# pasqal-io/pulser-diff

Measured on AMD Instinct MI355X. Metric: time-steps/sec (fwd+grad), higher is better.
Workload: dtype c128; 1 GPU; c3: 20-qubit register, 1000 time steps, fwd+grad wrt 8 pulse params per parameter set, KRYLOV_SE map, 1 parameter set(s) in the job; n_qubits=20, trajectories_total=1, trajectories_this_rank=1, ranks=1, gathered_parameter_sets=1, parallelism=trajectory-sharded x1 (one replica per rank), kernel_family=chained-tiles, tape=full

## Files before the change

pulser-diff_amd/csrc/pair_kernels.hpp:

```cpp
#pragma once

struct Chain2Args {
    const double2* v;
    const double2* w;
    const double2* t;
    double2* vmid_out;
    double2* y_out;
    double2* w_out;
    double2* t_out;
    const double* utt;
    const double* vr;
    const double* coef_fin;
    const double* coef_sta;
    long coef_bstride;
    double a_r, a_i, b_r, b_i, k_r, k_i;
    double g1_r, g1_i, b1_r, b1_i;
    int lo, hs, hb;
    uint32_t dim;
    int has_p, has_q;
    int gd;
    uint32_t fin_mask;
    uint32_t dmask[kMaxGroups];
    int dcnt[kMaxGroups];
    int b_first, b_count;
    const double* obs;
    double* expect_slot;
    int n_obs;
    long exp_ostride;
};

template <int LT, int LGT>
__global__ __launch_bounds__(1 << LGT) void k_chain2(Chain2Args a) {
    constexpr int NT = 1 << LGT, R = 1 << (LT - LGT);
    extern __shared__ __attribute__((aligned(16))) double2 tiles[];
    double* red = reinterpret_cast<double*>(tiles + 2 * (size_t(1) << LT));
    const unsigned tid = threadIdx.x;
    const unsigned t = blockIdx.x;
    const unsigned bl = blockIdx.y;
    if (bl >= unsigned(a.b_count)) return;
    const unsigned bt = unsigned(a.b_first) + bl;
    const size_t boff = size_t(bt) * a.dim;
    const unsigned lomask = (1u << a.lo) - 1u;
    const int midlow = a.hs - a.lo;
    const unsigned xbase = ((t & ((1u << midlow) - 1u)) << a.lo) | ((t >> midlow) << (a.hs + a.hb));
    double2 uu[R], ww[R], tt[R];
    unsigned xg[R];
#pragma unroll
    for (int r = 0; r < R; ++r) {
        const unsigned i = unsigned(r) * NT + tid;
        xg[r] = xbase | (i & lomask) | ((i >> a.lo) << a.hs);
        uu[r] = stream_load(a.v + boff + xg[r]);
    }
#pragma unroll
    for (int r = 0; r < R; ++r) ww[r] = stream_load(a.w + boff + xg[r]);
#pragma unroll
    for (int r = 0; r < R; ++r) tt[r] = stream_load(a.t + boff + xg[r]);
    double du[R];
    {
        const double* __restrict__ vrow = a.vr + size_t(t) * 16;
        double vloc[LT];
#pragma unroll
        for (int b2 = 0; b2 < LT; ++b2) vloc[b2] = vrow[b2];
        double dlane = vrow[LT];
#pragma unroll
        for (int b2 = 0; b2 < LGT; ++b2)
            if (!(tid >> b2 & 1u)) dlane += vloc[b2];
#pragma unroll
        for (int r = 0; r < R; ++r) {
            double d = a.utt[unsigned(r) * NT + tid] + dlane;
#pragma unroll
            for (int b2 = LGT; b2 < LT; ++b2)
                if (!(r >> (b2 - LGT) & 1)) d += vloc[b2];
            du[r] = d;
        }
    }
    auto diag = [&](const double* cf, int r) -> double {
        double d = du[r];
        for (int g = 0; g < a.gd; ++g) d += cf[2 + g] * double(a.dcnt[g] - popc_i(xg[r] & a.dmask[g]));
        return d;
    };
    int buf = 0;
    auto put = [&](const double2 (&val)[R]) -> const double2* {
        double2* tile = tiles + (size_t(buf) << LT);
#pragma unroll
        for (int r = 0; r < R; ++r) tile[unsigned(r) * NT + tid] = val[r];
        __syncthreads();
        buf ^= 1;
        return tile;
    };
    auto cmul = [](double xr, double xi, const double2& z) { return make_double2(xr * z.x - xi * z.y, xr * z.y + xi * z.x); };

    double2 y[R];
    if (a.has_p) {
        const double* __restrict__ cf = a.coef_fin + bt * a.coef_bstride;
        const double c = cf[0];
        double2 s[R], h1[R], ds[R];
        partner_sums<LT, LGT, false>(put(uu), uu, a.fin_mask, tid, s, ds);
        double d[R];
#pragma unroll
        for (int r = 0; r < R; ++r) {
            d[r] = diag(cf, r);
            h1[r].x = d[r] * uu[r].x + c * (ww[r].x + s[r].x);
            h1[r].y = d[r] * uu[r].y + c * (ww[r].y + s[r].y);
            const double2 p = cmul(a.a_r, a.a_i, uu[r]), q = cmul(a.b_r, a.b_i, h1[r]);
            y[r] = make_double2(p.x + q.x, p.y + q.y);
        }
        if (a.vmid_out) {
#pragma unroll
            for (int r = 0; r < R; ++r) {
                const double2 p = cmul(a.g1_r, a.g1_i, uu[r]), q = cmul(a.b1_r, a.b1_i, h1[r]);
                stream_store(a.vmid_out + boff + xg[r], make_double2(p.x + q.x, p.y + q.y));
            }
        }
        if (a.k_r != 0.0 || a.k_i != 0.0) {
            double2 e[R], pe[R];
#pragma unroll
            for (int r = 0; r < R; ++r) e[r] = make_double2(h1[r].x + c * ww[r].x, h1[r].y + c * ww[r].y);
            partner_sums<LT, LGT, false>(put(e), e, a.fin_mask, tid, pe, ds);
#pragma unroll
            for (int r = 0; r < R; ++r) {
                const double2 z = make_double2(d[r] * h1[r].x + c * (tt[r].x + pe[r].x), d[r] * h1[r].y + c * (tt[r].y + pe[r].y));
                const double2 k = cmul(a.k_r, a.k_i, z);
                y[r].x += k.x;
                y[r].y += k.y;
            }
        }
#pragma unroll
        for (int r = 0; r < R; ++r) stream_store(a.y_out + boff + xg[r], y[r]);
        if (a.obs) {
            for (int o = 0; o < a.n_obs; ++o) {
                double ex = 0.0;
#pragma unroll
                for (int r = 0; r < R; ++r) ex += a.obs[size_t(o) * a.dim + xg[r]] * (y[r].x * y[r].x + y[r].y * y[r].y);
                wg_atomic_add<NT>(ex, a.expect_slot + o * a.exp_ostride + bt, red);
            }
        }
    } else {
#pragma unroll
        for (int r = 0; r < R; ++r) y[r] = uu[r];
    }
    if (!a.has_q) return;

    const double* __restrict__ cf = a.coef_sta + bt * a.coef_bstride;
    const double c = cf[0];
    double2 w2[R], ds[R];
    partner_sums<LT, LGT, false, true>(put(y), y, ~0u, tid, w2, ds);
#pragma unroll
    for (int r = 0; r < R; ++r) stream_store(a.w_out + boff + xg[r], w2[r]);
    double2 z[R];
#pragma unroll
    for (int r = 0; r < R; ++r) {
        const double d = diag(cf, r);
        z[r] = make_double2(d * y[r].x + c * w2[r].x, d * y[r].y + c * w2[r].y);
    }
    double2 t2[R];
    partner_sums<LT, LGT, false, true>(put(z), z, ~0u, tid, t2, ds);
#pragma unroll
    for (int r = 0; r < R; ++r) stream_store(a.t_out + boff + xg[r], t2[r]);
}

struct Chain2BwdArgs {
    const double2* mu;
    const double2* w;
    const double2* t;
    const double2* xa;
    const double2* xb;
    double2* mu_out;
    double2* w_out;
    double2* t_out;
    const double* utt;
    const double* vr;
    const double* coef_fin;
    const double* coef_sta;
    long coef_bstride;
    double gb_r, gb_i, bb_r, bb_i;
    double k_r, k_i;
    double ga_r, ga_i, ba_r, ba_i;
    double cba_r, cba_i, cbb_r, cbb_i;
    int lo, hs, hb;
    uint32_t dim;
    int has_p, has_q;
    int gd;
    uint32_t fin_mask;
    uint32_t dmask;
    int dcnt;
    int b_first, b_count;
    double* ge_fin;
    long ge_bstride, ge_rstride;
    int det_slot;
    double* wtot;
    const double2* inj_gstate;
    const double* inj_gexp;
    const double* inj_obs;
    int inj_n_obs;
    long inj_ostride;
};

template <int LT, int LGT>
__global__ __launch_bounds__(1 << LGT) void k_chain2_bwd(Chain2BwdArgs a) {
    constexpr int NT = 1 << LGT, R = 1 << (LT - LGT), NW = NT / 64;
    extern __shared__ __attribute__((aligned(16))) double2 tiles[];
    double* red = reinterpret_cast<double*>(tiles + 2 * (size_t(1) << LT));
    const unsigned tid = threadIdx.x;
    const unsigned t = blockIdx.x;
    const unsigned bl = blockIdx.y;
    if (bl >= unsigned(a.b_count)) return;
    const unsigned bt = unsigned(a.b_first) + bl;
    const size_t boff = size_t(bt) * a.dim;
    const unsigned lomask = (1u << a.lo) - 1u;
    const int midlow = a.hs - a.lo;
    const unsigned xbase = ((t & ((1u << midlow) - 1u)) << a.lo) | ((t >> midlow) << (a.hs + a.hb));
    if (tid < 2 * NW) red[tid] = 0.0;
    double2 uu[R], ww[R], xa[R], xb[R], tp[R];
    unsigned xg[R];
    auto reindex = [&]() {
        unsigned tid_o = tid;
        asm volatile("" : "+v"(tid_o));
#pragma unroll
        for (int r = 0; r < R; ++r) {
            const unsigned i = unsigned(r) * NT + tid_o;
            xg[r] = xbase | (i & lomask) | ((i >> a.lo) << a.hs);
        }
    };
#pragma unroll
    for (int r = 0; r < R; ++r) {
        const unsigned i = unsigned(r) * NT + tid;
        xg[r] = xbase | (i & lomask) | ((i >> a.lo) << a.hs);
        uu[r] = stream_load(a.mu + boff + xg[r]);
    }
#pragma unroll
    for (int r = 0; r < R; ++r) ww[r] = stream_load(a.w + boff + xg[r]);
#pragma unroll
    for (int r = 0; r < R; ++r) xa[r] = stream_load(a.xa + boff + xg[r]);
    auto interaction_diagonal = [&](double (&du)[R]) {
        unsigned tid_o = tid;
        asm volatile("" : "+v"(tid_o));
        const double* __restrict__ vrow = a.vr + size_t(t) * 16;
        double vloc[LT];
#pragma unroll
        for (int b2 = 0; b2 < LT; ++b2) vloc[b2] = vrow[b2];
        double dlane = vrow[LT];
#pragma unroll
        for (int b2 = 0; b2 < LGT; ++b2)
            if (!(tid >> b2 & 1u)) dlane += vloc[b2];
#pragma unroll
        for (int r = 0; r < R; ++r) {
            double d = a.utt[unsigned(r) * NT + tid_o] + dlane;
#pragma unroll
            for (int b2 = LGT; b2 < LT; ++b2)
                if (!(r >> (b2 - LGT) & 1)) d += vloc[b2];
            du[r] = d;
        }
    };
    double du[R];
    interaction_diagonal(du);
    auto cnt = [&](int r) -> double { return a.gd ? double(a.dcnt - popc_i(xg[r] & a.dmask)) : 0.0; };
    int buf = 0;
    auto put = [&](const double2 (&val)[R]) -> const double2* {
        double2* tile = tiles + (size_t(buf) << LT);
#pragma unroll
        for (int r = 0; r < R; ++r) tile[unsigned(r) * NT + tid] = val[r];
        __syncthreads();
        buf ^= 1;
        return tile;
    };
    auto cmul = [](double xr, double xi, const double2& z) { return make_double2(xr * z.x - xi * z.y, xr * z.y + xi * z.x); };
    auto cdot = [](const double2& p, const double2& x) { return make_double2(p.x * x.x + p.y * x.y, p.x * x.y - p.y * x.x); };

    double2 y[R];
    if (a.has_p) {
        const double* __restrict__ cf = a.coef_fin + bt * a.coef_bstride;
        const double c = cf[0], cdet = a.gd ? cf[2] : 0.0;
        double2 pm[R], mid[R];
        double wx[R];
        double zc = 0.0;
        const bool two = a.k_r != 0.0 || a.k_i != 0.0;
        {
            double2* etile = tiles + (size_t(buf ^ 1) << LT);
#pragma unroll
            for (int r = 0; r < R; ++r) etile[unsigned(r) * NT + tid] = xa[r];
            double2 s[R], ds[R];
            partner_sums<LT, LGT, false>(put(uu), uu, a.fin_mask, tid, s, ds);
#pragma unroll
            for (int r = 0; r < R; ++r) {
                const double2 xav = etile[unsigned(r) * NT + tid];
                const double d = du[r] + cdet * cnt(r);
                pm[r] = make_double2(ww[r].x + s[r].x, ww[r].y + s[r].y);
                const double2 h1 = make_double2(d * uu[r].x + c * pm[r].x, d * uu[r].y + c * pm[r].y);
                if (two) etile[unsigned(r) * NT + tid] = make_double2(h1.x + c * ww[r].x, h1.y + c * ww[r].y);
                const double2 q1 = cdot(pm[r], xav);
                zc += a.cba_r * q1.x - a.cba_i * q1.y;
                const double2 wa = cdot(uu[r], xav);
                wx[r] = a.cba_r * wa.x - a.cba_i * wa.y;
                const double2 mm = cmul(a.ga_r, a.ga_i, uu[r]), mh = cmul(a.ba_r, a.ba_i, h1);
                mid[r] = make_double2(mm.x + mh.x, mm.y + mh.y);
            }
        }
        park1<NW>(zc, red, 0);
        zc = 0.0;
#pragma unroll
        for (int r = 0; r < R; ++r) xb[r] = stream_load(a.xb + boff + xg[r]);
#pragma unroll
        for (int r = 0; r < R; ++r) tp[r] = stream_load(a.t + boff + xg[r]);
        reindex();
        double sgd = 0.0;
#pragma unroll
        for (int r = 0; r < R; ++r) {
            const double2 wb = cdot(mid[r], xb[r]);
            const double wr = wx[r] + (a.cbb_r * wb.x - a.cbb_i * wb.y);
            if (a.wtot) unsafeAtomicAdd(a.wtot + xg[r], wr);
            sgd += wr * cnt(r);
            const double2 gpm = cmul(a.ga_r, a.ga_i, pm[r]);
            const double2 q = cdot(gpm, xb[r]);
            zc += a.cbb_r * q.x - a.cbb_i * q.y;
            const double d = du[r] + cdet * cnt(r);
            const double2 y1 = cmul(a.gb_r + a.bb_r * d, a.gb_i + a.bb_i * d, mid[r]), y2 = cmul(a.bb_r * c, a.bb_i * c, gpm);
            y[r] = make_double2(y1.x + y2.x, y1.y + y2.y);
        }
        __builtin_amdgcn_sched_barrier(0);
        if (two) {
            __syncthreads();
            buf ^= 1;
        }
        if (two) {
            const double2* tile = tiles + (size_t(buf ^ 1) << LT);
#pragma unroll
            for (int b = 0; b < LT; ++b) {
                if (a.fin_mask >> b & 1u) {
#pragma unroll
                    for (int r = 0; r < R; ++r) {
                        const double2 q = tile[(unsigned(r) * NT + tid) ^ (1u << b)];
                        tp[r].x += q.x;
                        tp[r].y += q.y;
                    }
                }
            }
        }
        const double kc_r = a.k_r * c, kc_i = a.k_i * c;
#pragma unroll
        for (int r = 0; r < R; ++r) {
            const double2 kt = cmul(kc_r, kc_i, tp[r]);
            y[r].x += kt.x;
            y[r].y += kt.y;
            const double2 q = cdot(cmul(a.ba_r, a.ba_i, tp[r]), xb[r]);
            zc += a.cbb_r * q.x - a.cbb_i * q.y;
        }
        park2<NW>(zc, sgd, red, 0, 1);
        reindex();
        if (a.inj_gexp || a.inj_gstate) {
            if (a.inj_gexp) {
                bool any = false;
                for (int o = 0; o < a.inj_n_obs; ++o) any |= a.inj_gexp[o * a.inj_ostride + bt] != 0.0;
                if (any) {
#pragma unroll
                    for (int r = 0; r < R; ++r) {
                        double wsum = 0.0;
                        for (int o = 0; o < a.inj_n_obs; ++o) wsum += a.inj_gexp[o * a.inj_ostride + bt] * a.inj_obs[size_t(o) * a.dim + xg[r]];
                        y[r].x += 2.0 * wsum * xb[r].x;
                        y[r].y += 2.0 * wsum * xb[r].y;
                    }
                }
            }
            if (a.inj_gstate) {
#pragma unroll
                for (int r = 0; r < R; ++r) {
                    const double2 gs = stream_load(a.inj_gstate + boff + xg[r]);
                    y[r].x += gs.x;
                    y[r].y += gs.y;
                }
            }
        }
#pragma unroll
        for (int r = 0; r < R; ++r) stream_store(a.mu_out + boff + xg[r], y[r]);
    } else {
#pragma unroll
        for (int r = 0; r < R; ++r) y[r] = uu[r];
    }
    auto flush = [&]() {
        if (a.has_p && tid < 2) {
            double sum = 0.0;
#pragma unroll
            for (int w = 0; w < NW; ++w) sum += red[tid * NW + w];
            double* ge = a.ge_fin + bt * a.ge_bstride + (blockIdx.x % kGradReplicas) * a.ge_rstride;
            if (sum != 0.0) unsafeAtomicAdd(ge + (tid ? a.det_slot : 0), sum);
        }
    };
    if (!a.has_q) {
        __syncthreads();
        flush();
        return;
    }

    const double* __restrict__ cf = a.coef_sta + bt * a.coef_bstride;
    const double c = cf[0], cdet = a.gd ? cf[2] : 0.0;
    reindex();
    interaction_diagonal(du);
    double2 w2[R], ds[R];
    partner_sums<LT, LGT, false, true>(put(y), y, ~0u, tid, w2, ds);
#pragma unroll
    for (int r = 0; r < R; ++r) stream_store(a.w_out + boff + xg[r], w2[r]);
    double2 z[R];
#pragma unroll
    for (int r = 0; r < R; ++r) {
        const double d = du[r] + cdet * cnt(r);
        z[r] = make_double2(d * y[r].x + c * w2[r].x, d * y[r].y + c * w2[r].y);
    }
    double2 t2[R];
    partner_sums<LT, LGT, false, true>(put(z), z, ~0u, tid, t2, ds);
#pragma unroll
    for (int r = 0; r < R; ++r) stream_store(a.t_out + boff + xg[r], t2[r]);
    flush();
}
```

pulser-diff_amd/csrc/pair_launch.hpp:

```cpp
#pragma once

namespace {

bool pair_legal(const Runtime& rt) {
    const Plan& pl = rt.pl;
    const uint32_t all = uint32_t(pl.dim) - 1u;
    const ChainGeom g = chain_geom(rt);
    return rt.pair_mode >= 0 && rt.variant == 0 && !rt.force_three && !rt.force_xcd && chain_enabled(rt) && !pl.shard_bits &&
           pl.N > kTileBits && pl.N <= 20 && g.lt == kTileBits && g.layouts == 2 && pl.ga.n == 1 && pl.gd.n <= 1 && !pl.ga.flagged &&
           (pl.ga.amp_index_mask[0] & all) == all && !(rt.flags & 1) && pl.off_pp2 && pl.off_pp3;
}

bool pair_enabled(const Runtime& rt) {
    if (!pair_legal(rt)) return false;
    return rt.pair_mode == 1 || (rt.pl.N == 20 && rt.pl.B == 1);
}

template <class Args>
void fill_chain2(Args& ca, const Runtime& rt, char* ws, const std::vector<ChainItem>& items, const std::vector<std::pair<int, int>>& blk,
                 int j, const double2* cur, const BatchSlice& bs) {
    const Plan& pl = rt.pl;
    double2* wt[2][2] = {{reinterpret_cast<double2*>(ws + pl.off_pp0), reinterpret_cast<double2*>(ws + pl.off_pp1)},
                         {reinterpret_cast<double2*>(ws + pl.off_pp2), reinterpret_cast<double2*>(ws + pl.off_pp3)}};
    const ChainGeom geom{kTileBits, 2};
    const int nb = int(blk.size()), L = j & 1;
    const LayoutDesc Y = chain_layout(pl.NL, L, geom), X = chain_layout(pl.NL, L ^ 1, geom);
    ca.w = j ? wt[(j - 1) & 1][0] : cur;
    ca.t = j ? wt[(j - 1) & 1][1] : cur;
    ca.utt = split_tables(pl, ws, kTileBits) + size_t(L) * rt.per_layout(kTileBits);
    ca.vr = ca.utt + (size_t(1) << kTileBits);
    ca.coef_bstride = rt.coef_bstride();
    ca.coef_fin = rt.coef(ws, j ? items[blk[j - 1].first].stage : 0);
    ca.coef_sta = rt.coef(ws, j < nb ? items[blk[j].first].stage : 0);
    ca.lo = Y.lo;
    ca.hs = Y.hs;
    ca.hb = Y.hb;
    ca.dim = uint32_t(pl.dim);
    ca.has_p = j > 0;
    ca.has_q = j < nb;
    ca.gd = pl.gd.n;
    ca.b_first = bs.first;
    ca.b_count = bs.count;
    if (ca.has_p) ca.fin_mask = to_tile_mask(Y, kTileBits, uint32_t(pl.dim - 1) & ~X.bits);
    if (ca.has_q) {
        ca.w_out = wt[j & 1][0];
        ca.t_out = wt[j & 1][1];
    }
}

template <int LGT>
int launch_chain2_t(const Chain2Args& ca, unsigned tiles, hipStream_t stream) {
    constexpr int LT = kTileBits;
    const size_t lds = 2 * (size_t(1) << LT) * sizeof(double2) + 256;
    if (int rc = set_max_dynamic_lds_once<&k_chain2<LT, LGT>>(lds)) return rc;
    hipLaunchKernelGGL((k_chain2<LT, LGT>), dim3(tiles, unsigned(ca.b_count)), dim3(1 << LGT), lds, stream, ca);
    LAUNCH_CHECK();
    return RYDIFF_OK;
}

template <class DstFn, class DoneFn, class ExpFn>
int run_chain2(const Runtime& rt, char* ws, const std::vector<ChainItem>& items, const double2* start, DstFn dst, bool keep_mid,
               DoneFn on_done, ExpFn exp_slot, const BatchSlice& bs, hipStream_t stream) {
    const Plan& pl = rt.pl;
    const int F = int(items.size());
    if (F <= 0) return RYDIFF_OK;
    std::vector<std::pair<int, int>> blk;
    for (int i = 0; i < F;) {
        if (i + 1 < F && items[i + 1].stage == items[i].stage) {
            blk.push_back({i, i + 1});
            i += 2;
        } else {
            blk.push_back({i, -1});
            ++i;
        }
    }
    const unsigned tiles = unsigned(pl.dim >> kTileBits);
    const int nb = int(blk.size());
    const double2* cur = start;
    for (int j = 0; j <= nb; ++j) {
        Chain2Args ca{};
        fill_chain2(ca, rt, ws, items, blk, j, cur, bs);
        ca.v = cur;
        fill_detuning(ca.dmask, ca.dcnt, pl);
        int f0 = -1, last = -1;
        if (ca.has_p) {
            f0 = blk[j - 1].first;
            const int f1 = blk[j - 1].second;
            last = f1 >= 0 ? f1 : f0;
            const FactorScalars& s1 = items[f0].s;
            const FactorScalars s2 = f1 >= 0 ? items[f1].s : FactorScalars{1.0, 0.0, 0.0, 0.0};
            const std::complex<double> g1(s1.gr, s1.gi), b1(s1.br, s1.bi), g2(s2.gr, s2.gi), b2(s2.br, s2.bi);
            const std::complex<double> qa = g1 * g2, qb = g1 * b2 + b1 * g2, qk = b1 * b2;
            ca.a_r = qa.real();
            ca.a_i = qa.imag();
            ca.b_r = qb.real();
            ca.b_i = qb.imag();
            ca.k_r = qk.real();
            ca.k_i = qk.imag();
            ca.g1_r = s1.gr;
            ca.g1_i = s1.gi;
            ca.b1_r = s1.br;
            ca.b1_i = s1.bi;
            ca.vmid_out = (f1 >= 0 && keep_mid) ? dst(f0) : nullptr;
            ca.y_out = dst(last);
            if (!ca.y_out) return fail(RYDIFF_EINVAL, "internal: chain destination missing");
            ChainStep cs{};
            exp_slot(last, cs);
            ca.obs = cs.obs;
            ca.expect_slot = cs.expect_slot;
            ca.n_obs = cs.n_obs;
            ca.exp_ostride = cs.exp_ostride;
        }
        int rc = launch_chain2_t<10>(ca, tiles, stream);
        if (rc) return rc;
        if (ca.has_p) {
            if (ca.vmid_out) {
                rc = on_done(f0, ca.vmid_out);
                if (rc) return rc;
            }
            rc = on_done(last, ca.y_out);
            if (rc) return rc;
            cur = ca.y_out;
        }
    }
    return RYDIFF_OK;
}

bool pair_bwd_enabled(const Runtime& rt) {
    const ChainGeom g = chain_geom(rt);
    return !rt.pair_bwd_off && rt.real_amp_grad && pair_enabled(rt) && g.lt == kTileBits && g.layouts == 2;
}

template <int LGT>
int launch_chain2_bwd_t(const Chain2BwdArgs& ca, unsigned tiles, hipStream_t stream) {
    constexpr int LT = kTileBits;
    const size_t lds = 2 * (size_t(1) << LT) * sizeof(double2) + 2 * ((size_t(1) << LGT) / 64) * sizeof(double);
    if (int rc = set_max_dynamic_lds_once<&k_chain2_bwd<LT, LGT>>(lds)) return rc;
    hipLaunchKernelGGL((k_chain2_bwd<LT, LGT>), dim3(tiles, unsigned(ca.b_count)), dim3(1 << LGT), lds, stream, ca);
    LAUNCH_CHECK();
    return RYDIFF_OK;
}

template <class StageEndFn>
int run_chain2_bwd(const Runtime& rt, char* ws, const std::vector<ChainItem>& items, const std::vector<const double2*>& xs,
                   const std::vector<int>& save_k, const double2* lam_in, double2* lam_bufs[2], int& cl, double* wtot,
                   StageEndFn on_stage_end, const BatchSlice& bs, const InjectSource& inj, hipStream_t stream) {
    const Plan& pl = rt.pl;
    const int M = int(items.size());
    if (M <= 0) return RYDIFF_OK;
    std::vector<std::pair<int, int>> blk;
    for (int f = M - 1; f >= 0;) {
        if (f >= 1 && items[f - 1].stage == items[f].stage) {
            blk.push_back({f - 1, f});
            f -= 2;
        } else {
            blk.push_back({f, -1});
            --f;
        }
    }
    const unsigned tiles = unsigned(pl.dim >> kTileBits);
    const int nb = int(blk.size());
    const double2* cur = lam_in;
    int rc = on_stage_end(items[M - 1].stage, cur, xs[M]);
    if (rc) return rc;
    for (int j = 0; j <= nb; ++j) {
        Chain2BwdArgs ca{};
        fill_chain2(ca, rt, ws, items, blk, j, cur, bs);
        ca.mu = cur;
        ca.xa = ca.xb = cur;
        if (pl.gd.n) {
            ca.dmask = pl.gd.amp_index_mask[0];
            ca.dcnt = pl.gd.count[0];
        }
        ca.ge_fin = rt.ge(ws, 0);
        ca.ge_bstride = rt.ge_bstride();
        ca.ge_rstride = pl.NC + 1;
        ca.det_slot = 2 * pl.ga.n;
        ca.wtot = wtot;
        int fb = -1;
        if (ca.has_p) {
            fb = blk[j - 1].first;
            const int fa = blk[j - 1].second;
            const FactorScalars& sb = items[fb].s;
            const FactorScalars sa = fa >= 0 ? items[fa].s : FactorScalars{1.0, 0.0, 0.0, 0.0};
            const std::complex<double> gb(sb.gr, -sb.gi), bb(sb.br, -sb.bi), ga(sa.gr, -sa.gi), ba(sa.br, -sa.bi);
            const std::complex<double> qk = ba * bb;
            ca.gb_r = gb.real();
            ca.gb_i = gb.imag();
            ca.bb_r = bb.real();
            ca.bb_i = bb.imag();
            ca.k_r = qk.real();
            ca.k_i = qk.imag();
            ca.ga_r = ga.real();
            ca.ga_i = ga.imag();
            ca.ba_r = ba.real();
            ca.ba_i = ba.imag();
            ca.cba_r = sa.br;
            ca.cba_i = sa.bi;
            ca.cbb_r = sb.br;
            ca.cbb_i = sb.bi;
            ca.xb = xs[fb];
            ca.xa = fa >= 0 ? xs[fa] : xs[fb];
            ca.ge_fin = rt.ge(ws, items[fb].stage);
            cl ^= 1;
            ca.mu_out = lam_bufs[cl];
            if (ca.mu_out == cur) return fail(RYDIFF_EINVAL, "internal: cotangent ping-pong clash");
            fill_inject(ca, inj, save_k[fb], pl);
        }
        rc = launch_chain2_bwd_t<10>(ca, tiles, stream);
        if (rc) return rc;
        if (ca.has_p) {
            cur = ca.mu_out;
            if (fb >= 1 && items[fb].stage != items[fb - 1].stage) {
                rc = on_stage_end(items[fb - 1].stage, cur, xs[fb]);
                if (rc) return rc;
            }
        }
    }
    return RYDIFF_OK;
}

}
```

pulser-diff_amd/csrc/rydiff.hip:

```cpp
#include <hip/hip_runtime.h>

#include <algorithm>
#include <atomic>
#include <complex>
#include <cstdio>
#include <cstdlib>
#include <cstring>
#include <functional>
#include <mutex>
#include <type_traits>
#include <string>
#include <vector>

#include "../../include/rydiff.h"
#include "plan.hpp"
#include "poly.hpp"

using namespace rydiff;

#include "common.hpp"
#include "direct_kernels.hpp"
#include "chain_kernels.hpp"
#include "pair_kernels.hpp"
#include "persist_kernels.hpp"
#include "lane_kernels.hpp"
#include "pauli_kernels.hpp"
static_assert(sizeof(PersistFactor) == 48, "plan.hpp sizes the factor table with 48 bytes per entry");

#include "runtime.hpp"
#include "pauli_launch.hpp"
#include "direct_launch.hpp"
#include "chain_launch.hpp"
#include "pair_launch.hpp"
#include "persist_launch.hpp"

namespace {

void describe_kernels(const Runtime& rt, const RydProblem* p, bool backward, RydPlanInfo* info) {
    const Plan& pl = rt.pl;
    auto b = [](bool v) { return v ? "true" : "false"; };
    info->kernel_fwd[0] = info->kernel_bwd[0] = 0;
    if (info->kernel_family == 3) {
        const bool pairs = pl.tape_mode != 3 && xcd_group_size(rt, false) == 0 && pair_enabled(rt);
        const bool pairs_bwd = xcd_group_size(rt, true) == 0 && pair_bwd_enabled(rt);
        const bool fast = pl.ga.n == 1 && (pl.ga.amp_index_mask[0] & ((1u << pl.NL) - 1u)) == (1u << pl.NL) - 1u && !pl.ga.flagged;
        for (int bwd = 0; bwd <= (backward ? 1 : 0); ++bwd) {
            const bool cplx = (rt.flags & 1) != 0 || (bwd && !p->real_amp_grad);
            const int lgt = rt.variant == 0 ? ((bwd && cplx) ? 9 : 10) : rt.chain_lgt;
            const bool res = xcd_group_size(rt, bwd != 0) > 0;
            if (!bwd && pairs)
                std::snprintf(info->kernel_fwd, sizeof(info->kernel_fwd), "k_chain2<%d,10>", kTileBits);
            else if (bwd && pairs_bwd)
                std::snprintf(info->kernel_bwd, sizeof(info->kernel_bwd), "k_chain2_bwd<%d,10>", kTileBits);
            else if (chain_geom(rt).lt == kWideTileBits)
                std::snprintf(bwd ? info->kernel_bwd : info->kernel_fwd, sizeof(info->kernel_fwd), "k_chain_wide<%d,%s,%s,%s>", kWideTileBits,
                              b(cplx), b(bwd != 0), b(fast));
            else
                std::snprintf(bwd ? info->kernel_bwd : info->kernel_fwd, sizeof(info->kernel_fwd), "k_chain<%d,%d,%s,%s,%s,%s>", chain_geom(rt).lt,
                              chain_geom(rt).lt == kTileBits ? lgt : 10, b(cplx), b(bwd != 0), b(fast), b(res));
        }
    } else if (info->kernel_family == 2) {
        if (direct_global_ok(rt)) {
            std::snprintf(info->kernel_fwd, sizeof(info->kernel_fwd), "k_factor_direct_global<%d,%s>", pl.N, b(pl.N <= 13));
            if (backward) std::snprintf(info->kernel_bwd, sizeof(info->kernel_bwd), "k_factor_bwd_direct_global<%d,%s>", pl.N, b(pl.N <= 13));
        } else {
            std::snprintf(info->kernel_fwd, sizeof(info->kernel_fwd), "k_factor_direct");
            if (backward) std::snprintf(info->kernel_bwd, sizeof(info->kernel_bwd), "k_factor_bwd_direct");
        }
    } else {
        std::snprintf(info->kernel_fwd, sizeof(info->kernel_fwd), info->kernel_family == 0 ? "k_lanes_fwd (N=%d)" : "k_persist<%d,...>", pl.N);
        if (backward) std::snprintf(info->kernel_bwd, sizeof(info->kernel_bwd), info->kernel_family == 0 ? "k_lanes_bwd (N=%d)" : "k_persist_bwd<%d,...>", pl.N);
    }
}

int launch_expect(const ForwardCtx& c, const double2* psi, int k) {
    const Plan& pl = c.rt.pl;
    const unsigned red_blocks = unsigned(std::min<size_t>((pl.dim + 255) / 256, 1024));
    hipLaunchKernelGGL(k_expect_diag, dim3(red_blocks, pl.B), dim3(256), 0, c.stream, psi, c.obs, c.expect_out, pl.n_obs, pl.T + 1, k, pl.B,
                       uint32_t(pl.dim), c.rt.obs_bstride());
    LAUNCH_CHECK();
    return RYDIFF_OK;
}

int forward_chained(const ForwardCtx& c) {
    const Runtime& rt = c.rt;
    const Plan& pl = rt.pl;
    const size_t sv = c.sv;
    hipStream_t stream = c.stream;
    std::vector<ChainItem> all, chain;
    std::vector<int> step_of_end;
    std::vector<int64_t> b_entry;
    for (int k = 0; k < pl.T; ++k) {
        build_step_chain(rt, k, chain);
        for (size_t i = 0; i < chain.size(); ++i) {
            all.push_back(chain[i]);
            step_of_end.push_back(i + 1 == chain.size() ? k + 1 : 0);
            if (c.partial_tape()) b_entry.push_back((k >= c.tmap.k0 && i + 1 < chain.size()) ? c.tmap.bprefix[k] + int64_t(i) : -1);
        }
    }
    const int grp = xcd_group_size(rt, false);
    for (int b0 = 0; b0 < pl.B; b0 += (grp ? grp : pl.B)) {
        const BatchSlice bs{b0, std::min(grp ? grp : pl.B, pl.B - b0), grp > 0};
        int flip = 0;
        auto dst = [&](int i) -> double2* {
            if (c.full_tape()) return c.tape + size_t(i + 1) * sv;
            if (step_of_end[i] && c.tape) return c.tape + size_t(step_of_end[i]) * sv;
            if (c.partial_tape() && b_entry[i] >= 0) return c.tape_b + size_t(b_entry[i]) * sv;
            if (bs.xcd) return c.buf[0];
            flip ^= 1;
            return c.buf[flip];
        };
        auto done = [&](int i, const double2* out) -> int {
            if (c.final_dst && step_of_end[i] == pl.T)
                HIP_TRY(hipMemcpyAsync(c.final_dst + size_t(bs.first) * pl.dim, out + size_t(bs.first) * pl.dim,
                                       size_t(bs.count) * pl.dim * sizeof(double2), hipMemcpyDeviceToDevice, stream));
            if (c.copy_out && step_of_end[i])
                HIP_TRY(hipMemcpyAsync(c.copy_out + size_t(step_of_end[i]) * sv + size_t(bs.first) * pl.dim, out + size_t(bs.first) * pl.dim,
                                       size_t(bs.count) * pl.dim * sizeof(double2), hipMemcpyDeviceToDevice, stream));
            if (step_of_end[i]) return launch_pauli_expect(c, out, 0, step_of_end[i], 1, bs);
            return RYDIFF_OK;
        };
        auto exp_slot = [&](int i, ChainStep& cs) {
            if (c.want_exp && step_of_end[i]) {
                cs.obs = c.obs;
                cs.n_obs = pl.n_obs;
                cs.exp_ostride = long(pl.T + 1) * pl.B;
                cs.expect_slot = c.expect_out + size_t(step_of_end[i]) * pl.B;
            }
        };
        const int rc = (!c.partial_tape() && !bs.xcd && pair_enabled(rt))
                           ? run_chain2(rt, c.ws, all, c.start, dst, c.full_tape(), done, exp_slot, bs, stream)
                           : run_chain(rt, c.ws, all, c.start, dst, done, exp_slot, false, bs, stream);
        if (rc) return rc;
    }
    return RYDIFF_OK;
}

int forward_direct(const ForwardCtx& c) {
    const Runtime& rt = c.rt;
    const Plan& pl = rt.pl;
    const size_t sv = c.sv;
    std::vector<ChainItem> chain;
    const double2* cur = c.start;
    int pp = 0;
    bool exp_fused = false;
    size_t gfac = 0;
    for (int k = 0; k < pl.T; ++k) {
        build_step_chain(rt, k, chain);
        for (size_t i = 0; i < chain.size(); ++i, ++gfac) {
            const bool last = (i + 1 == chain.size());
            double2* dst;
            if (c.full_tape() && c.tape) dst = c.tape + (gfac + 1) * sv;
            else if (last && c.tape) dst = c.tape + size_t(k + 1) * sv;
            else if (c.partial_tape() && k >= c.tmap.k0) dst = c.tape_b + size_t(c.tmap.bprefix[k] + int64_t(i)) * sv;
            else {
                dst = c.buf[pp];
                if (dst == cur) dst = c.buf[pp ^ 1];
                pp ^= 1;
            }
            const bool want_here = c.want_exp && last;
            int rc = shard_signal(rt, 0, cur);
            if (!rc) rc = shard_signal(rt, 1, nullptr);
            if (rc) return rc;
            rc = launch_factor(rt, c.ws, cur, dst, chain[i].stage, chain[i].s, c.stream, want_here ? c.obs : nullptr,
                               want_here ? c.expect_out + size_t(k + 1) * pl.B : nullptr, &exp_fused);
            if (rc) return rc;
            cur = dst;
        }
        if (c.copy_out) HIP_TRY(hipMemcpyAsync(c.copy_out + size_t(k + 1) * sv, cur, pl.state_bytes, hipMemcpyDeviceToDevice, c.stream));
        if (c.want_exp && !exp_fused) {
            const int rc = launch_expect(c, cur, k + 1);
            if (rc) return rc;
        }
        if (const int rc = launch_pauli_expect(c, cur, 0, k + 1, 1, BatchSlice{0, pl.B, false})) return rc;
    }
    if (c.final_dst) HIP_TRY(hipMemcpyAsync(c.final_dst, cur, pl.state_bytes, hipMemcpyDeviceToDevice, c.stream));
    return RYDIFF_OK;
}

int gather_factor_inputs(const BackwardCtx& c, const BatchSlice& bs, int k, int k_hi, const std::vector<ChainItem>& chain,
                         std::vector<const double2*>& xs) {
    const Runtime& rt = c.rt;
    const int M = int(chain.size());
    const size_t sv = c.sv;
    xs.assign(M + 1, nullptr);
    xs[0] = c.state_at(k);
    xs[M] = c.state_at(k_hi + 1);
    if (c.full_tape()) {
        for (int i = 1; i < M; ++i) xs[i] = c.tape + size_t(c.fprefix[k] + i) * sv;
    } else if (c.taped(k_hi)) {
        int i = 0;
        for (int kk = k; kk <= k_hi; ++kk) {
            const int mk = int(c.fprefix[kk + 1] - c.fprefix[kk]);
            for (int j = 0; j < mk; ++j, ++i) xs[i] = j == 0 ? c.state_at(kk) : c.tape_b + size_t(c.tmap.bprefix[kk] + j - 1) * sv;
        }
    } else if (M - 1 > rt.pl.chain_slots) {
        return fail(RYDIFF_EWORKSPACE, "internal: chain buffers too small");
    } else if (chain_enabled(rt) && M > 1) {
        for (int i = 1; i < M; ++i) xs[i] = c.chainbuf + size_t(i - 1) * sv;
        auto dst = [&](int i) -> double2* { return c.chainbuf + size_t(i) * sv; };
        auto done = [&](int, const double2*) -> int { return RYDIFF_OK; };
        auto no_exp = [&](int, ChainStep&) {};
        return run_chain(rt, c.ws, chain, xs[0], dst, done, no_exp, true, bs, c.stream);
    } else {
        for (int i = 1; i < M; ++i) {
            double2* dst = c.chainbuf + size_t(i - 1) * sv;
            int rc = shard_signal(rt, 0, xs[i - 1]);
            if (!rc) rc = shard_signal(rt, 1, nullptr);
            if (rc) return rc;
            rc = launch_factor(rt, c.ws, xs[i - 1], dst, chain[i - 1].stage, chain[i - 1].s, c.stream);
            if (rc) return rc;
            xs[i] = dst;
        }
    }
    return RYDIFF_OK;
}

int adjoint_chained(const BackwardCtx& c, const BatchSlice& bs, const std::vector<ChainItem>& chain, const std::vector<const double2*>& xs,
                    const std::vector<int>& save_k, int& cl) {
    const Runtime& rt = c.rt;
    double2* lam[2] = {c.lam[0], c.lam[1]};
    auto dot_h = [&](int stage, const double2* g, const double2* xout) -> int {
        return c.want_tau ? launch_dot_h(rt, c.ws, stage, g, xout, bs, c.stream) : RYDIFF_OK;
    };
    return (!bs.xcd && pair_bwd_enabled(rt)) ? run_chain2_bwd(rt, c.ws, chain, xs, save_k, lam[cl], lam, cl, c.wtot, dot_h, bs, c.inj, c.stream)
                                             : run_chain_bwd(rt, c.ws, chain, xs, save_k, lam[cl], lam, cl, c.wtot, dot_h, c.want_tau, bs, c.inj, c.stream);
}

int adjoint_direct(const BackwardCtx& c, const BatchSlice& bs, const std::vector<ChainItem>& chain, const std::vector<const double2*>& xs,
                   const std::vector<int>& save_k, int& cl) {
    const Runtime& rt = c.rt;
    const int M = int(chain.size());
    for (int i = M; i >= 1; --i) {
        const ChainItem& it = chain[i - 1];
        int rc = shard_signal(rt, 0, c.lam[cl]);
        if (!rc) rc = shard_signal(rt, 1, nullptr);
        if (rc) return rc;
        if (c.want_tau && (i == M || chain[i].stage != it.stage)) {
            rc = launch_dot_h(rt, c.ws, it.stage, c.lam[cl], xs[i], bs, c.stream);
            if (rc) return rc;
        }
        rc = launch_factor_bwd(rt, c.ws, c.lam[cl], xs[i - 1], c.lam[cl ^ 1], it.stage, it.s, c.wtot, c.inj, save_k[i - 1], c.stream);
        if (rc) return rc;
        cl ^= 1;
    }
    return RYDIFF_OK;
}

int adjoint_sweep(const BackwardCtx& c, const BatchSlice& bs, int& cl) {
    const Runtime& rt = c.rt;
    const Plan& pl = rt.pl;
    const bool chained = chain_enabled(rt);
    std::vector<ChainItem> chain, part;
    std::vector<const double2*> xs;
    std::vector<int> save_k;
    cl = 0;
    for (int k = pl.T - 1; k >= 0; --k) {
        const int k_hi = k;
        if (c.taped(k_hi) && chained) {
            while (k > 0 && c.taped(k - 1) && c.fprefix[k_hi + 1] - c.fprefix[k - 1] < (int64_t(1) << 16)) --k;
        }
        chain.clear();
        save_k.clear();
        for (int kk = k; kk <= k_hi; ++kk) {
            build_step_chain(rt, kk, part);
            for (size_t i = 0; i < part.size(); ++i) save_k.push_back(i == 0 ? kk : -1);
            chain.insert(chain.end(), part.begin(), part.end());
        }
        int rc = gather_factor_inputs(c, bs, k, k_hi, chain, xs);
        if (!rc) rc = chained ? adjoint_chained(c, bs, chain, xs, save_k, cl) : adjoint_direct(c, bs, chain, xs, save_k, cl);
        if (rc) return rc;
    }
    return RYDIFF_OK;
}

int scatter_gradients(const BackwardCtx& c, void* g_amp, double* g_det, double* g_u, double* g_tsave) {
    const Plan& pl = c.rt.pl;
    hipStream_t stream = c.stream;
    const size_t E = pl.stages.size();
    if (g_amp) HIP_TRY(hipMemsetAsync(g_amp, 0, size_t(pl.Bc) * pl.Ka * pl.n_samples * 16, stream));
    if (g_det) HIP_TRY(hipMemsetAsync(g_det, 0, size_t(pl.Bc) * pl.Kd * pl.n_samples * 8, stream));
    if (g_tsave) HIP_TRY(hipMemsetAsync(g_tsave, 0, size_t(pl.T + 1) * 8, stream));
    if ((g_amp && pl.Ka) || (g_det && pl.Kd) || g_tsave) {
        char* m = c.ws + pl.off_meta2;
        if (g_tsave) {
            std::vector<StageBwdDev> sb(E);
            for (size_t e = 0; e < E; ++e) {
                const Stage& st = pl.stages[e];
                sb[e] = {st.tau_scale, st.tnw[0], st.tnw[1], st.tn[0], st.tn[1], st.t_hi, st.t_lo};
            }
            const int rc = upload_words(stream, m, sb.data(), E * sizeof(StageBwdDev));
            if (rc) return rc;
        }
        ScatterArgs sa{};
        sa.ge = c.ge;
        sa.st = reinterpret_cast<const StageDev*>(c.ws + pl.off_meta_idx);
        sa.sb = reinterpret_cast<const StageBwdDev*>(m);
        sa.inv_dt = pl.dt > 0.0 ? 1.0 / pl.dt : 0.0;
        sa.amp = static_cast<const double2*>(c.p->amp_tables);
        sa.det = c.p->det_tables;
        sa.g_amp = static_cast<double2*>(g_amp);
        sa.g_det = g_det;
        sa.g_tsave = g_tsave;
        sa.E = int(E);
        sa.n_samples = pl.n_samples;
        sa.Ka = pl.Ka;
        sa.Kd = pl.Kd;
        sa.NC = pl.NC;
        sa.ga = pl.ga.n;
        sa.gd = pl.gd.n;
        for (int g = 0; g < pl.ga.n; ++g) sa.amem[g] = pl.ga.members[g];
        for (int g = 0; g < pl.gd.n; ++g) sa.dmem[g] = pl.gd.members[g];
        hipLaunchKernelGGL(k_scatter_grads, dim3((unsigned(E) + 63) / 64, pl.Bc), dim3(64), 0, stream, sa);
        LAUNCH_CHECK();
    }
    const int npairs = pl.N * (pl.N - 1) / 2;
    if (g_u && npairs > 0) {
        HIP_TRY(hipMemsetAsync(g_u, 0, size_t(npairs) * 8, stream));
        const unsigned nb = unsigned(std::min<size_t>((pl.dim + 255) / 256, 256));
        hipLaunchKernelGGL(k_ugrad, dim3(nb, npairs), dim3(256), 0, stream, g_u, c.wtot, pl.N, uint32_t(pl.dim), pl.shard_bits ? pl.B : 0, pl.NL,
                           pl.rank_first);
        LAUNCH_CHECK();
    }
    return RYDIFF_OK;
}

}

extern "C" {

const char* rydiff_last_error(void) { return g_last_error.c_str(); }
const char* rydiff_version(void) { return "rydiff 0.4 (gfx950)"; }
size_t rydiff_sizeof_problem(void) { return sizeof(RydProblem); }
size_t rydiff_sizeof_plan_info(void) { return sizeof(RydPlanInfo); }

#ifdef RYDIFF_TIMELINE
int rydiff_debug_timeline(unsigned long long* host_buf, int n_entries) {
    return hipMemcpyFromSymbol(host_buf, HIP_SYMBOL(g_timeline), size_t(n_entries) * sizeof(unsigned long long)) == hipSuccess ? 0 : -3;
}
#endif

int rydiff_design_polynomial(double rho, double tol, int max_degree, int* degree, double* roots_reim, double* p0_reim, double* max_err) {
    if (!(rho > 0.0) || !degree || !roots_reim || max_degree < 1) return fail(RYDIFF_EINVAL, "bad arguments");
    PolyDesign d = design_polynomial(rho, tol, max_degree);
    if (d.degree < 1) return fail(RYDIFF_EINVAL, "polynomial design failed");
    *degree = d.degree;
    for (int i = 0; i < d.degree; ++i) {
        roots_reim[2 * i] = d.roots[i].real();
        roots_reim[2 * i + 1] = d.roots[i].imag();
    }
    if (p0_reim) {
        p0_reim[0] = d.p0.real();
        p0_reim[1] = d.p0.imag();
    }
    if (max_err) *max_err = d.max_err;
    return RYDIFF_OK;
// ... 208 lines not shown
```

Baseline: 4228 time-steps/s.

## Split pair backward kernel into FIRST variant and reorder loads for latency overlap

Templates k_chain2_bwd on a FIRST flag so the has_p=false case runs a lean start-only kernel, and removes the runtime has_p branches from the main path. All global loads (xa, w, xb, t) are issued up front behind sched barriers, and the utt table load is split from the diagonal computation so memory latency overlaps compute. Coefficient and interaction tables are read through the constant address space (scalar loads), and 32-bit byte-offset addressing is used. It also adds timeline probe hooks and raises register pressure by holding xb/tp live longer, which may lower occupancy.

```diff
diff --git a/pulser-diff_amd/csrc/pair_kernels.hpp b/pulser-diff_amd/csrc/pair_kernels.hpp
--- a/pulser-diff_amd/csrc/pair_kernels.hpp
+++ b/pulser-diff_amd/csrc/pair_kernels.hpp
@@ -196,7 +196,7 @@
     long inj_ostride;
 };
 
-template <int LT, int LGT>
+template <int LT, int LGT, bool FIRST>
 __global__ __launch_bounds__(1 << LGT) void k_chain2_bwd(Chain2BwdArgs a) {
     constexpr int NT = 1 << LGT, R = 1 << (LT - LGT), NW = NT / 64;
     extern __shared__ __attribute__((aligned(16))) double2 tiles[];
@@ -222,38 +222,44 @@
             xg[r] = xbase | (i & lomask) | ((i >> a.lo) << a.hs);
         }
     };
+    auto at = [&](auto* base, unsigned x) {
+        using char_t = std::conditional_t<std::is_const_v<std::remove_pointer_t<decltype(base)>>, const char, char>;
+        return reinterpret_cast<decltype(base)>(reinterpret_cast<char_t*>(base + boff) + unsigned(x << 4));
+    };
+    using ctab = const __attribute__((address_space(4))) double*;
+    auto request_tables = [&](double (&du)[R]) {
+        unsigned tid_o = tid;
+        asm volatile("" : "+v"(tid_o));
+#pragma unroll
+        for (int r = 0; r < R; ++r) du[r] = a.utt[unsigned(r) * NT + tid_o];
+    };
+    auto interaction_diagonal = [&](double (&du)[R]) {
+        ctab vrow = (ctab)(a.vr + size_t(t) * 16);
+        double vloc[LT];
+#pragma unroll
+        for (int b2 = 0; b2 < LT; ++b2) vloc[b2] = vrow[b2];
+        double dlane = vrow[LT];
+#pragma unroll
+        for (int b2 = 0; b2 < LGT; ++b2)
+            if (!(tid >> b2 & 1u)) dlane += vloc[b2];
+#pragma unroll
+        for (int r = 0; r < R; ++r) {
+            double d = du[r] + dlane;
+#pragma unroll
+            for (int b2 = LGT; b2 < LT; ++b2)
+                if (!(r >> (b2 - LGT) & 1)) d += vloc[b2];
+            du[r] = d;
+        }
+    };
+    RYDIFF_TL(0);
+    double du[R];
+    request_tables(du);
 #pragma unroll
     for (int r = 0; r < R; ++r) {
         const unsigned i = unsigned(r) * NT + tid;
         xg[r] = xbase | (i & lomask) | ((i >> a.lo) << a.hs);
-        uu[r] = stream_load(a.mu + boff + xg[r]);
-    }
-#pragma unroll
-    for (int r = 0; r < R; ++r) ww[r] = stream_load(a.w + boff + xg[r]);
-#pragma unroll
-    for (int r = 0; r < R; ++r) xa[r] = stream_load(a.xa + boff + xg[r]);
-    auto interaction_diagonal = [&](double (&du)[R]) {
-        unsigned tid_o = tid;
-        asm volatile("" : "+v"(tid_o));
-        const double* __restrict__ vrow = a.vr + size_t(t) * 16;
-        double vloc[LT];
-#pragma unroll
-        for (int b2 = 0; b2 < LT; ++b2) vloc[b2] = vrow[b2];
-        double dlane = vrow[LT];
-#pragma unroll
-        for (int b2 = 0; b2 < LGT; ++b2)
-            if (!(tid >> b2 & 1u)) dlane += vloc[b2];
-#pragma unroll
-        for (int r = 0; r < R; ++r) {
-            double d = a.utt[unsigned(r) * NT + tid_o] + dlane;
-#pragma unroll
-            for (int b2 = LGT; b2 < LT; ++b2)
-                if (!(r >> (b2 - LGT) & 1)) d += vloc[b2];
-            du[r] = d;
-        }
-    };
-    double du[R];
-    interaction_diagonal(du);
+        uu[r] = stream_load(at(a.mu, xg[r]));
+    }
     auto cnt = [&](int r) -> double { return a.gd ? double(a.dcnt - popc_i(xg[r] & a.dmask)) : 0.0; };
     int buf = 0;
     auto put = [&](const double2 (&val)[R]) -> const double2* {
@@ -267,9 +273,46 @@
     auto cmul = [](double xr, double xi, const double2& z) { return make_double2(xr * z.x - xi * z.y, xr * z.y + xi * z.x); };
     auto cdot = [](const double2& p, const double2& x) { return make_double2(p.x * x.x + p.y * x.y, p.x * x.y - p.y * x.x); };
 
+    auto start_block = [&](const double2 (&y)[R]) {
+        ctab cf = (ctab)(a.coef_sta + bt * a.coef_bstride);
+        const double c = cf[0], cdet = a.gd ? cf[2] : 0.0;
+        double2 w2[R], ds[R];
+        partner_sums<LT, LGT, false, true>(put(y), y, ~0u, tid, w2, ds);
+#pragma unroll
+        for (int r = 0; r < R; ++r) stream_store(at(a.w_out, xg[r]), w2[r]);
+        double2 z[R];
+#pragma unroll
+        for (int r = 0; r < R; ++r) {
+            const double d = du[r] + cdet * cnt(r);
+            z[r] = make_double2(d * y[r].x + c * w2[r].x, d * y[r].y + c * w2[r].y);
+        }
+        double2 t2[R];
+        partner_sums<LT, LGT, false, true>(put(z), z, ~0u, tid, t2, ds);
+#pragma unroll
+        for (int r = 0; r < R; ++r) stream_store(at(a.t_out, xg[r]), t2[r]);
+    };
+    if constexpr (FIRST) {
+        interaction_diagonal(du);
+        if (a.has_q) start_block(uu);
+        return;
+    }
+    __builtin_amdgcn_sched_barrier(0);
+#pragma unroll
+    for (int r = 0; r < R; ++r) xa[r] = stream_load(at(a.xa, xg[r]));
+    __builtin_amdgcn_sched_barrier(0);
+#pragma unroll
+    for (int r = 0; r < R; ++r) ww[r] = stream_load(at(a.w, xg[r]));
+    __builtin_amdgcn_sched_barrier(0);
+#pragma unroll
+    for (int r = 0; r < R; ++r) xb[r] = stream_load(at(a.xb, xg[r]));
+    __builtin_amdgcn_sched_barrier(0);
+#pragma unroll
+    for (int r = 0; r < R; ++r) tp[r] = stream_load(at(a.t, xg[r]));
+    __builtin_amdgcn_sched_barrier(0);
+    interaction_diagonal(du);
     double2 y[R];
-    if (a.has_p) {
-        const double* __restrict__ cf = a.coef_fin + bt * a.coef_bstride;
+    {
+        ctab cf = (ctab)(a.coef_fin + bt * a.coef_bstride);
         const double c = cf[0], cdet = a.gd ? cf[2] : 0.0;
         double2 pm[R], mid[R];
         double wx[R];
@@ -280,7 +323,9 @@
 #pragma unroll
             for (int r = 0; r < R; ++r) etile[unsigned(r) * NT + tid] = xa[r];
             double2 s[R], ds[R];
-            partner_sums<LT, LGT, false>(put(uu), uu, a.fin_mask, tid, s, ds);
+            const double2* utile = put(uu);
+            RYDIFF_TL(1);
+            partner_sums<LT, LGT, false>(utile, uu, a.fin_mask, tid, s, ds);
 #pragma unroll
             for (int r = 0; r < R; ++r) {
                 const double2 xav = etile[unsigned(r) * NT + tid];
@@ -298,10 +343,7 @@
         }
         park1<NW>(zc, red, 0);
         zc = 0.0;
-#pragma unroll
-        for (int r = 0; r < R; ++r) xb[r] = stream_load(a.xb + boff + xg[r]);
-#pragma unroll
-        for (int r = 0; r < R; ++r) tp[r] = stream_load(a.t + boff + xg[r]);
+        RYDIFF_TL(2);
         reindex();
         double sgd = 0.0;
 #pragma unroll
@@ -318,6 +360,7 @@
             y[r] = make_double2(y1.x + y2.x, y1.y + y2.y);
         }
         __builtin_amdgcn_sched_barrier(0);
+        RYDIFF_TL(3);
         if (two) {
             __syncthreads();
             buf ^= 1;
@@ -346,6 +389,7 @@
             zc += a.cbb_r * q.x - a.cbb_i * q.y;
         }
         park2<NW>(zc, sgd, red, 0, 1);
+        RYDIFF_TL(4);
         reindex();
         if (a.inj_gexp || a.inj_gstate) {
             if (a.inj_gexp) {
@@ -364,20 +408,20 @@
             if (a.inj_gstate) {
 #pragma unroll
                 for (int r = 0; r < R; ++r) {
-                    const double2 gs = stream_load(a.inj_gstate + boff + xg[r]);
+                    const double2 gs = stream_load(at(a.inj_gstate, xg[r]));
                     y[r].x += gs.x;
                     y[r].y += gs.y;
                 }
             }
         }
-#pragma unroll
-        for (int r = 0; r < R; ++r) stream_store(a.mu_out + boff + xg[r], y[r]);
-    } else {
-#pragma unroll
-        for (int r = 0; r < R; ++r) y[r] = uu[r];
+        request_tables(du);
+#pragma unroll
+        for (int r = 0; r < R; ++r) stream_store(at(a.mu_out, xg[r]), y[r]);
+        RYDIFF_TL(5);
+        interaction_diagonal(du);
     }
     auto flush = [&]() {
-        if (a.has_p && tid < 2) {
+        if (tid < 2) {
             double sum = 0.0;
 #pragma unroll
             for (int w = 0; w < NW; ++w) sum += red[tid * NW + w];
@@ -390,24 +434,11 @@
         flush();
         return;
     }
-
-    const double* __restrict__ cf = a.coef_sta + bt * a.coef_bstride;
-    const double c = cf[0], cdet = a.gd ? cf[2] : 0.0;
-    reindex();
-    interaction_diagonal(du);
-    double2 w2[R], ds[R];
-    partner_sums<LT, LGT, false, true>(put(y), y, ~0u, tid, w2, ds);
-#pragma unroll
-    for (int r = 0; r < R; ++r) stream_store(a.w_out + boff + xg[r], w2[r]);
-    double2 z[R];
-#pragma unroll
-    for (int r = 0; r < R; ++r) {
-        const double d = du[r] + cdet * cnt(r);
-        z[r] = make_double2(d * y[r].x + c * w2[r].x, d * y[r].y + c * w2[r].y);
-    }
-    double2 t2[R];
-    partner_sums<LT, LGT, false, true>(put(z), z, ~0u, tid, t2, ds);
-#pragma unroll
-    for (int r = 0; r < R; ++r) stream_store(a.t_out + boff + xg[r], t2[r]);
+    start_block(y);
+    RYDIFF_TL(6);
     flush();
+#ifdef RYDIFF_TIMELINE
+    __builtin_amdgcn_s_waitcnt(0);
+    RYDIFF_TL(7);
+#endif
 }
diff --git a/pulser-diff_amd/csrc/pair_launch.hpp b/pulser-diff_amd/csrc/pair_launch.hpp
--- a/pulser-diff_amd/csrc/pair_launch.hpp
+++ b/pulser-diff_amd/csrc/pair_launch.hpp
@@ -131,12 +131,12 @@
     return !rt.pair_bwd_off && rt.real_amp_grad && pair_enabled(rt) && g.lt == kTileBits && g.layouts == 2;
 }
 
-template <int LGT>
+template <int LGT, bool FIRST>
 int launch_chain2_bwd_t(const Chain2BwdArgs& ca, unsigned tiles, hipStream_t stream) {
     constexpr int LT = kTileBits;
     const size_t lds = 2 * (size_t(1) << LT) * sizeof(double2) + 2 * ((size_t(1) << LGT) / 64) * sizeof(double);
-    if (int rc = set_max_dynamic_lds_once<&k_chain2_bwd<LT, LGT>>(lds)) return rc;
-    hipLaunchKernelGGL((k_chain2_bwd<LT, LGT>), dim3(tiles, unsigned(ca.b_count)), dim3(1 << LGT), lds, stream, ca);
+    if (int rc = set_max_dynamic_lds_once<&k_chain2_bwd<LT, LGT, FIRST>>(lds)) return rc;
+    hipLaunchKernelGGL((k_chain2_bwd<LT, LGT, FIRST>), dim3(tiles, unsigned(ca.b_count)), dim3(1 << LGT), lds, stream, ca);
     LAUNCH_CHECK();
     return RYDIFF_OK;
 }
@@ -207,7 +207,10 @@
             if (ca.mu_out == cur) return fail(RYDIFF_EINVAL, "internal: cotangent ping-pong clash");
             fill_inject(ca, inj, save_k[fb], pl);
         }
-        rc = launch_chain2_bwd_t<10>(ca, tiles, stream);
+#ifndef RYDIFF_PAIR_BWD_LGT
+#define RYDIFF_PAIR_BWD_LGT 10
+#endif
+        rc = ca.has_p ? launch_chain2_bwd_t<RYDIFF_PAIR_BWD_LGT, false>(ca, tiles, stream) : launch_chain2_bwd_t<RYDIFF_PAIR_BWD_LGT, true>(ca, tiles, stream);
         if (rc) return rc;
         if (ca.has_p) {
             cur = ca.mu_out;
diff --git a/pulser-diff_amd/csrc/rydiff.hip b/pulser-diff_amd/csrc/rydiff.hip
--- a/pulser-diff_amd/csrc/rydiff.hip
+++ b/pulser-diff_amd/csrc/rydiff.hip
@@ -51,7 +51,7 @@
             if (!bwd && pairs)
                 std::snprintf(info->kernel_fwd, sizeof(info->kernel_fwd), "k_chain2<%d,10>", kTileBits);
             else if (bwd && pairs_bwd)
-                std::snprintf(info->kernel_bwd, sizeof(info->kernel_bwd), "k_chain2_bwd<%d,10>", kTileBits);
+                std::snprintf(info->kernel_bwd, sizeof(info->kernel_bwd), "k_chain2_bwd<%d,%d,false>", kTileBits, RYDIFF_PAIR_BWD_LGT);
             else if (chain_geom(rt).lt == kWideTileBits)
                 std::snprintf(bwd ? info->kernel_bwd : info->kernel_fwd, sizeof(info->kernel_fwd), "k_chain_wide<%d,%s,%s,%s>", kWideTileBits,
                               b(cplx), b(bwd != 0), b(fast));
```

Result: slower. 4121 time-steps/s (-2.5%).
